# jyakaranda/A-LeGO-LOAM

Measured on AMD Instinct MI355X. Metric: scans/sec (16x1800 LiDAR) full IP->LO->LM loop, higher is better.
Workload: dtype f32/f64

## Files before the change

### a-lego-loam_amd/binding.py

```python
import ctypes as C
import os

import numpy as np

from .params import AlegoParams, AlegoPoint

_HERE = os.path.dirname(os.path.abspath(__file__))
_lib = None
_DT = {0: np.float32, 1: np.float64, 2: np.int32, 3: np.uint8}

EXPORTS = [
    "alego_create", "alego_destroy", "alego_last_error", "alego_device_count", "alego_params_sizeof",
    "alego_ip_process", "alego_lo_process", "alego_lm_process", "alego_scan_process",
    "alego_batch_load", "alego_batch_run", "alego_synchronize", "alego_batch_get_pose", "alego_batch_get_counts",
    "alego_stream", "alego_stream_groups", "alego_profile_enable", "alego_profile_report", "alego_set_lo_params", "alego_set_lm_params", "alego_debug_get", "alego_debug_voxel", "alego_debug_atan2f",
    "alego_lo_push_imu", "alego_lo_get_undistorted", "alego_pose_o2b", "alego_trajectory_enable", "alego_trajectory_get", "alego_debug_check_guards", "alego_debug_math", "alego_debug_std_sort", "alego_debug_eval_blocks", "alego_debug_transform_to_start", "alego_debug_set_option",
    "alego_lm_keyframe_count", "alego_lm_get_keyframe", "alego_lm_set_keypose", "alego_lm_reset_window", "alego_lm_apply_correction",
    "alego_lm_add_keyframe", "alego_pc2_to_points", "alego_replay_create", "alego_replay_load", "alego_replay_assign",
    "alego_dist_unique_id", "alego_dist_init", "alego_dist_shutdown", "alego_dist_allreduce_probe", "alego_stream_setup", "alego_stream_run",
    "alego_loop_detect", "alego_loop_closure_icp",
    "alego_bag_open", "alego_bag_close", "alego_bag_last_error", "alego_bag_topic_count", "alego_bag_topic_info", "alego_bag_message_count",
    "alego_bag_read_raw", "alego_bag_read_pc2", "alego_handle_lock", "alego_handle_unlock",
    "alego_map_enable", "alego_map_status", "alego_map_set_keyposes", "alego_map_get_keyframe", "alego_map_assemble", "alego_map_keyposes",
    "alego_lm_get_local_map", "alego_voxel_grid", "alego_write_pcd",
    "alego_map_get_stamps", "alego_map_set_stamps", "alego_loop_search", "alego_loop_constraint", "alego_debug_nn1",
    "alego_graph_enable", "alego_graph_status", "alego_graph_get_edges", "alego_graph_set_edges", "alego_graph_add_loops", "alego_graph_add_edge",
    "alego_graph_optimize", "alego_graph_get_estimate", "alego_graph_residuals",
    "alego_loc_select", "alego_loc_enable", "alego_loc_status",
    "alego_reloc_enable", "alego_loc_relocalize", "alego_reloc_descriptor", "alego_reloc_match", "alego_debug_reloc_search",
    "alego_loop_appearance_enable", "alego_loop_search_appearance", "alego_loop_appearance_candidates",
    "alego_map_align", "alego_map_align_queries", "alego_map_align_consensus", "alego_map_align_poses",
    "alego_map_move", "alego_map_merge", "alego_map_align_edge", "alego_map_merge_edges",
    "alego_map_thin", "alego_map_thin_select", "alego_map_thin_edges", "alego_debug_thin_select",
]

REPLAY_PINGPONG = 0x100
REPLAY_BAG = 0x200
MAP_SURF, MAP_CORNER, MAP_OUTLIER, MAP_FRAME_ID = 1, 2, 4, 8
ERR_CAPACITY, ERR_ARG = -3, -4
RELOC_MAX_CAND = 8
RELOC_SECTORS, RELOC_RINGS = 60, 20
ALIGN_MAX_QUERIES = 32
ALIGN_TOL_TRANS, ALIGN_TOL_ROT = 0.24, 0.0165
MERGE_COPY_ITEM = 1024
FLAG_LO_INIT, FLAG_FEW_SURF, FLAG_FEW_CORNER, FLAG_LM_SKIPPED, FLAG_LM_FEW_FEATURES, FLAG_LM_KEYFRAME = 1, 2, 4, 8, 16, 32


class ScanIn(C.Structure):
    _fields_ = [("pts", C.c_void_p), ("n", C.c_int32), ("stamp", C.c_double)]


class SegOut(C.Structure):
    _fields_ = [("seg", C.c_void_p), ("seg_cap", C.c_int32), ("m", C.c_int32),
                ("ground", C.c_void_p), ("col", C.c_void_p), ("range", C.c_void_p),
                ("ring_start", C.c_void_p), ("ring_end", C.c_void_p), ("orientation", C.c_float * 3),
                ("outlier", C.c_void_p), ("outlier_cap", C.c_int32), ("n_outlier", C.c_int32),
                ("label_image", C.c_void_p), ("stamp", C.c_double)]


class FeatOut(C.Structure):
    _fields_ = [("sharp", C.c_void_p), ("sharp_cap", C.c_int32), ("n_sharp", C.c_int32),
                ("less_sharp", C.c_void_p), ("less_sharp_cap", C.c_int32), ("n_less_sharp", C.c_int32),
                ("flat", C.c_void_p), ("flat_cap", C.c_int32), ("n_flat", C.c_int32),
                ("less_flat", C.c_void_p), ("less_flat_cap", C.c_int32), ("n_less_flat", C.c_int32),
                ("point_label", C.c_void_p)]


class Pose(C.Structure):
# ... 142 lines not shown


class Pc2Field(C.Structure):
    _fields_ = [("name", C.c_char_p), ("offset", C.c_uint32), ("datatype", C.c_uint8), ("count", C.c_uint32)]


def lib_path():
    return os.environ.get("ALEGO_LIB") or os.path.join(_HERE, "libalego_mi355x.so")


def lib():
    global _lib
    if _lib is None:
        path = lib_path()
        if not os.path.exists(path):
            raise RuntimeError(f"{path} missing: the HIP extension is not built (run __graft_entry__.build()); "
                               "there is no CPU fallback")
        L = C.CDLL(path)
        L.alego_create.restype = C.c_int
        L.alego_create.argtypes = [C.POINTER(AlegoParams), C.c_int, C.c_int, C.c_int, C.POINTER(C.c_void_p)]
        L.alego_destroy.argtypes = [C.c_void_p]
        L.alego_last_error.restype = C.c_char_p
        L.alego_last_error.argtypes = [C.c_void_p]
        L.alego_device_count.restype = C.c_int
        L.alego_params_sizeof.restype = C.c_int
        L.alego_ip_process.restype = C.c_int
        L.alego_ip_process.argtypes = [C.c_void_p, C.POINTER(ScanIn), C.POINTER(SegOut)]
        L.alego_lo_process.restype = C.c_int
        L.alego_lo_process.argtypes = [C.c_void_p, C.POINTER(SegOut), C.POINTER(FeatOut), C.POINTER(Pose)]
        L.alego_lm_process.restype = C.c_int
        L.alego_lm_process.argtypes = [C.c_void_p, C.c_void_p, C.c_int32, C.c_void_p, C.c_int32, C.c_void_p, C.c_int32,
                                       C.POINTER(Pose), C.POINTER(Pose)]
        L.alego_scan_process.restype = C.c_int
        L.alego_scan_process.argtypes = [C.c_void_p, C.c_int, C.POINTER(ScanIn), C.c_int, C.POINTER(SegOut),
                                         C.POINTER(FeatOut), C.POINTER(Pose), C.POINTER(Pose)]
        L.alego_batch_load.restype = C.c_int
        L.alego_batch_load.argtypes = [C.c_void_p, C.c_int, C.c_int, C.c_void_p, C.c_int32]
        L.alego_batch_run.restype = C.c_int
        L.alego_batch_run.argtypes = [C.c_void_p, C.c_int, C.c_int, C.c_int, C.c_int]
        L.alego_synchronize.restype = C.c_int
        L.alego_synchronize.argtypes = [C.c_void_p]
        L.alego_batch_get_pose.restype = C.c_int
        L.alego_batch_get_pose.argtypes = [C.c_void_p, C.c_int, C.POINTER(Pose), C.POINTER(Pose)]
        L.alego_batch_get_counts.restype = C.c_int
        L.alego_batch_get_counts.argtypes = [C.c_void_p, C.c_int, C.c_void_p, C.c_int]
        L.alego_profile_enable.restype = C.c_int
        L.alego_profile_enable.argtypes = [C.c_void_p, C.c_int]
        L.alego_profile_report.restype = C.c_int
        L.alego_profile_report.argtypes = [C.c_void_p, C.c_char_p, C.c_int, C.c_void_p, C.c_void_p, C.c_int]
        L.alego_stream.restype = C.c_void_p
        L.alego_stream.argtypes = [C.c_void_p]
        L.alego_stream_groups.restype = C.c_int
        L.alego_stream_groups.argtypes = [C.c_void_p, C.POINTER(C.c_int)]
        L.alego_set_lo_params.restype = C.c_int
        L.alego_set_lo_params.argtypes = [C.c_void_p, C.c_int, C.c_void_p]
        L.alego_set_lm_params.restype = C.c_int
        L.alego_set_lm_params.argtypes = [C.c_void_p, C.c_int, C.c_void_p]
        L.alego_debug_get.restype = C.c_int
        L.alego_debug_get.argtypes = [C.c_void_p, C.c_int, C.c_char_p, C.c_void_p, C.c_int, C.POINTER(C.c_int), C.POINTER(C.c_int)]
        L.alego_debug_voxel.restype = C.c_int
        L.alego_debug_voxel.argtypes = [C.c_void_p, C.c_void_p, C.c_int, C.c_float, C.c_void_p, C.c_int]
        L.alego_debug_atan2f.restype = C.c_int
        L.alego_debug_atan2f.argtypes = [C.c_void_p, C.c_void_p, C.c_void_p, C.c_void_p, C.c_int]
        L.alego_trajectory_enable.restype = C.c_int
        L.alego_trajectory_enable.argtypes = [C.c_void_p, C.c_int32]
        L.alego_trajectory_get.restype = C.c_int
        L.alego_trajectory_get.argtypes = [C.c_void_p, C.c_int, C.c_int32, C.c_int32, C.c_void_p]
        L.alego_lo_push_imu.restype = C.c_int
        L.alego_lo_push_imu.argtypes = [C.c_void_p, C.c_int, C.c_void_p, C.c_int32]
        L.alego_lo_get_undistorted.restype = C.c_int
        L.alego_lo_get_undistorted.argtypes = [C.c_void_p, C.c_int, C.c_void_p, C.c_int32]
        L.alego_pose_o2b.restype = C.c_int
        L.alego_pose_o2b.argtypes = [C.c_void_p, C.c_void_p, C.c_void_p]
        L.alego_debug_check_guards.restype = C.c_int
        L.alego_debug_check_guards.argtypes = [C.c_char_p, C.c_int]
        L.alego_debug_std_sort.restype = C.c_int
        L.alego_debug_std_sort.argtypes = [C.c_void_p, C.c_void_p, C.c_int, C.c_int, C.c_void_p]
        L.alego_debug_math.restype = C.c_int
        L.alego_debug_math.argtypes = [C.c_void_p, C.c_int, C.c_void_p, C.c_void_p, C.c_void_p, C.c_int]
        L.alego_debug_eval_blocks.restype = C.c_int
        L.alego_debug_eval_blocks.argtypes = [C.c_void_p, C.c_int, C.c_int, C.c_void_p, C.c_void_p, C.c_void_p, C.c_void_p]
        L.alego_debug_transform_to_start.restype = C.c_int
        L.alego_debug_transform_to_start.argtypes = [C.c_void_p, C.c_void_p, C.c_void_p, C.c_int, C.c_void_p]
        L.alego_debug_set_option.restype = C.c_int
        L.alego_debug_set_option.argtypes = [C.c_void_p, C.c_char_p, C.c_int]
        L.alego_lm_keyframe_count.restype = C.c_int
        L.alego_lm_keyframe_count.argtypes = [C.c_void_p, C.c_int]
        L.alego_lm_get_keyframe.restype = C.c_int
        L.alego_lm_get_keyframe.argtypes = [C.c_void_p, C.c_int, C.c_int, C.POINTER(KeyFrame)]
        L.alego_lm_set_keypose.restype = C.c_int
        L.alego_lm_set_keypose.argtypes = [C.c_void_p, C.c_int, C.c_int, C.c_void_p]
        L.alego_lm_reset_window.restype = C.c_int
        L.alego_lm_reset_window.argtypes = [C.c_void_p, C.c_int]
        L.alego_lm_apply_correction.restype = C.c_int
        L.alego_lm_apply_correction.argtypes = [C.c_void_p, C.c_int, C.c_void_p]
        L.alego_lm_add_keyframe.restype = C.c_int
        L.alego_lm_add_keyframe.argtypes = [C.c_void_p, C.c_int, C.c_void_p, C.c_void_p, C.c_int32, C.c_void_p, C.c_int32, C.c_void_p, C.c_int32]
        L.alego_pc2_to_points.restype = C.c_int
        L.alego_pc2_to_points.argtypes = [C.c_void_p, C.c_uint64, C.c_uint32, C.c_uint32, C.c_uint32, C.c_uint32, C.c_int,
                                          C.POINTER(Pc2Field), C.c_int, C.c_void_p, C.c_int32]
        L.alego_replay_create.restype = C.c_int
        L.alego_replay_create.argtypes = [C.c_void_p, C.c_int, C.c_int]
        L.alego_replay_load.restype = C.c_int
        L.alego_replay_load.argtypes = [C.c_void_p, C.c_int, C.c_int, C.c_void_p, C.c_int32]
        L.alego_replay_assign.restype = C.c_int
        L.alego_replay_assign.argtypes = [C.c_void_p, C.c_int, C.c_int, C.c_int]
# ... 479 lines not shown

    def replay_create(self, n_bags, bag_len):
        self._check(lib().alego_replay_create(self._h, n_bags, bag_len), "alego_replay_create")

    def replay_load(self, bag, scan, pts):
        a = np.ascontiguousarray(pts, dtype=np.float32)
        self._check(lib().alego_replay_load(self._h, bag, scan, a.ctypes.data, a.shape[0]), "alego_replay_load")

    def replay_assign(self, slot, bag, start_scan):
        self._check(lib().alego_replay_assign(self._h, slot, bag, start_scan), "alego_replay_assign")

    def stream_setup(self, bag, start_scan=0):
        self._check(lib().alego_stream_setup(self._h, bag, start_scan), "alego_stream_setup")

    def stream_run(self, first_step, n_scans, stages=7, sync=True):
        self._check(lib().alego_stream_run(self._h, first_step, n_scans, stages, 1 if sync else 0), "alego_stream_run")

    def batch_run(self, first_pos, n_scans, stages=7, sync=True):
        self._check(lib().alego_batch_run(self._h, first_pos, n_scans, stages, 1 if sync else 0), "alego_batch_run")

    def synchronize(self):
        self._check(lib().alego_synchronize(self._h), "alego_synchronize")

    def batch_get_pose(self, slot=0):
        odom, mp = Pose(), Pose()
        flags = self._check(lib().alego_batch_get_pose(self._h, slot, C.byref(odom), C.byref(mp)), "alego_batch_get_pose")
        return flags, odom.as_dict(), mp.as_dict()

    def batch_get_counts(self, slot=0):
        out = np.zeros(16, np.int32)
        self._check(lib().alego_batch_get_counts(self._h, slot, out.ctypes.data, 16), "alego_batch_get_counts")
        keys = ["P", "M", "O", "Qc", "Fc", "Qs", "Fs", "n_surf_corr", "n_corner_corr", "Kraw_c", "Kraw_s", "Kds_c", "Kds_s", "Lc", "Ls", "n_rebuild"]
        return dict(zip(keys, out.tolist()))

    def profile_enable(self, on=True):
        self._check(lib().alego_profile_enable(self._h, 1 if on else 0), "alego_profile_enable")

    def profile_report(self):
        names = C.create_string_buffer(8192)
        tot = np.zeros(256, np.float64)
        cnt = np.zeros(256, np.int32)
        n = self._check(lib().alego_profile_report(self._h, names, 8192, tot.ctypes.data, cnt.ctypes.data, 256), "alego_profile_report")
        ks = names.value.decode().split(";") if n else []
        return {k: (float(tot[i]), int(cnt[i])) for i, k in enumerate(ks)}

    def stream(self):
        return lib().alego_stream(self._h)

    def stream_groups(self):
        per = C.c_int(0)
        g = lib().alego_stream_groups(self._h, C.byref(per))
        return g, per.value

    def set_lo_params(self, p6, slot=0):
        a = np.ascontiguousarray(p6, np.float64)
        self._check(lib().alego_set_lo_params(self._h, slot, a.ctypes.data), "alego_set_lo_params")

    def set_lm_params(self, p6, slot=0):
        a = np.ascontiguousarray(p6, np.float64)
        self._check(lib().alego_set_lm_params(self._h, slot, a.ctypes.data), "alego_set_lm_params")

    def debug_get(self, name, slot=0, cap_bytes=None):
        cap = cap_bytes or max(self.N * 64 + 4096, 8 << 20)
        buf = np.empty(cap, np.uint8)
        cnt, dt = C.c_int(), C.c_int()
        self._check(lib().alego_debug_get(self._h, slot, name.encode(), buf.ctypes.data, cap, C.byref(cnt), C.byref(dt)),
                    f"alego_debug_get({name})")
        dtype = np.dtype(_DT[dt.value])
        out = np.frombuffer(buf.tobytes()[:cnt.value * dtype.itemsize], dtype=dtype).copy()
        return out.reshape(-1, 4) if (name in _CLOUDS or name.startswith("lm_") and name.endswith(("_ds", "_map"))) else out

    def voxel_grid(self, pts, leaf):
        a = np.ascontiguousarray(pts, np.float32)
        out = np.empty((max(a.shape[0], 1), 4), np.float32)
        n = self._check(lib().alego_debug_voxel(self._h, a.ctypes.data, a.shape[0], leaf, out.ctypes.data, out.shape[0]), "alego_debug_voxel")
        return out[:n].copy()

    def voxel_grid_large(self, pts, leaf):
        a = np.ascontiguousarray(pts, np.float32).reshape(-1, 4)
        n = self._check(lib().alego_voxel_grid(self._h, a.ctypes.data, a.shape[0], leaf, None, 0), "alego_voxel_grid")
        out = np.empty((max(n, 1), 4), np.float32)
        m = self._check(lib().alego_voxel_grid(self._h, a.ctypes.data, a.shape[0], leaf, out.ctypes.data, out.shape[0]), "alego_voxel_grid")
        return out[:m].copy()

    def map_enable(self, max_keyframes, max_points):
        self._check(lib().alego_map_enable(self._h, max_keyframes, max_points), "alego_map_enable")

    def map_status(self, slot=0):
        out = np.zeros(4, np.int32)
        self._check(lib().alego_map_status(self._h, slot, out.ctypes.data), "alego_map_status")
        return tuple(int(v) for v in out)

    def map_set_keyposes(self, first, poses6, slot=0):
        a = np.ascontiguousarray(poses6, np.float32).reshape(-1, 6)
        self._check(lib().alego_map_set_keyposes(self._h, slot, first, a.shape[0], a.ctypes.data), "alego_map_set_keyposes")

    def map_get_keyframe(self, kf_id, slot=0):
        k = KeyFrame()
        self._check(lib().alego_map_get_keyframe(self._h, slot, kf_id, C.byref(k)), "alego_map_get_keyframe")
        bufs = [np.empty((max(n, 1), 4), np.float32) for n in (k.n_corner, k.n_surf, k.n_outlier)]
        k.corner, k.corner_cap = bufs[0].ctypes.data, bufs[0].shape[0]
        k.surf, k.surf_cap = bufs[1].ctypes.data, bufs[1].shape[0]
        k.outlier, k.outlier_cap = bufs[2].ctypes.data, bufs[2].shape[0]
        self._check(lib().alego_map_get_keyframe(self._h, slot, kf_id, C.byref(k)), "alego_map_get_keyframe")
        return dict(id=int(k.id), pose=np.array(k.pose[:], np.float32), corner=bufs[0][:k.n_corner].copy(), surf=bufs[1][:k.n_surf].copy(),
                    outlier=bufs[2][:k.n_outlier].copy())
# ... 336 lines not shown
```

### a-lego-loam_amd/csrc/alego_api.hip

```cpp
#include <hip/hip_runtime.h>

#include <cmath>
#include <cstdio>
#include <cstdlib>
#include <algorithm>
#include <cstring>
#include <mutex>
#include <set>
#include <string>
#include <vector>

#include "../../include/alego_mi355x.h"
#include "dev_common.h"
#include "dev_mem.h"
#include "front_end.h"
#include "lm_ctx.h"
#include "lm_host.h"
#include "merge_math.h"
#include "thin_math.h"
#include "loop_ctx.h"
#include "pgraph.h"
#include "prof.h"
#include "reloc.h"
#include "voxel.h"

thread_local Profiler* g_prof = nullptr;


struct alego_handle {
  std::recursive_mutex host_lock;
  alego_params P;
  int device = 0;
  hipStream_t stream = nullptr;
  std::vector<hipStream_t> streams;
  int gsize = 1;
  bool lm_async = false;
  std::vector<hipStream_t> back;
  std::vector<hipEvent_t> ev_stage, ev_back;
  std::vector<long> grp_scans;
  DevCtx d;
  DevPool mem;
  std::string err;
  std::vector<long> lo_scans;
  LmHost* lm = nullptr;
  Profiler prof;
  int ip_fast_capable = 0;
  bool replay_assigned = false;
  bool stream_mode = false;
  int lanes = 0;
  int pose_slot = 0;
  int last_lane = -1;
  std::vector<double> imu_last_stamp;
  int next_set = 0;
  hipStream_t s_lo = nullptr, s_lm = nullptr;
  std::vector<hipEvent_t> ev_pool;
  size_t ev_next = 0;
  bool map_on = false;
  LcCtx* lc = nullptr;
  bool graph_on = false;
  PgCtx* pg = nullptr;
  RlCtx* rl = nullptr;
};

namespace {

#define HIP_TRY(h, call)                                                                       \
  do {                                                                                         \
    hipError_t e_ = (call);                                                                    \
    if (e_ != hipSuccess) {                                                                    \
      (h)->err = std::string(#call) + ": " + hipGetErrorString(e_);                            \
      return ALEGO_ERR_HIP;                                                                    \
    }                                                                                          \
  } while (0)

template <class T>
int dalloc(alego_handle* h, T** p, size_t count, bool zero = true) {
  const hipError_t e = h->mem.get(p, count, zero);
  if (e != hipSuccess) { h->err = std::string("device allocation: ") + hipGetErrorString(e); return ALEGO_ERR_HIP; }
  return 0;
}

DevCtx view(const alego_handle* h, int slot0, int n) {
  DevCtx d = h->d;
  d.slot0 = slot0;
  d.n_launch = n;
  return d;
}

hipStream_t stream_of(const alego_handle* h, int slot) { return h->streams[slot / h->gsize]; }
hipError_t sync_all(const alego_handle* h) {
  hipError_t r = hipSuccess;
  for (hipStream_t s : h->streams) { hipError_t e = hipStreamSynchronize(s); if (e != hipSuccess) r = e; }
  for (hipStream_t s : h->back) { hipError_t e = hipStreamSynchronize(s); if (e != hipSuccess) r = e; }
  for (hipStream_t s : {h->s_lo, h->s_lm}) if (s) { hipError_t e = hipStreamSynchronize(s); if (e != hipSuccess) r = e; }
  return r;
}

int env_int(const char* name, int dflt) { const char* e = getenv(name); return e ? atoi(e) : dflt; }

void drain_back(alego_handle* h, int slot = -1) {
  if (slot >= 0 && !h->back.empty()) { (void)hipStreamSynchronize(h->back[std::min<size_t>((size_t)(slot / h->gsize), h->back.size() - 1)]); return; }
  for (hipStream_t s : h->back) (void)hipStreamSynchronize(s);
}
int check_slot(alego_handle* h, int slot, bool drain = true) {
  if (!h) return ALEGO_ERR_ARG;
  if (slot < 0 || slot >= h->d.n_slots) { h->err = "slot out of range"; return ALEGO_ERR_ARG; }
  if (drain) drain_back(h, slot);
  return 0;
}

int not_localising(alego_handle* h, const char* what) {
  if (h->lm && lm_host_localising(h->lm)) { h->err = std::string(what) + ": not available on a localising handle (alego_loc_enable)"; return ALEGO_ERR_ARG; }
  return 0;
}

}

extern "C" {

int alego_device_count(void) {
  int n = 0;
  if (hipGetDeviceCount(&n) != hipSuccess) return 0;
  return n;
}
int alego_params_sizeof(void) { return (int)sizeof(alego_params); }
int alego_handle_lock(alego_handle* h) { if (!h) return ALEGO_ERR_ARG; h->host_lock.lock(); return 0; }
int alego_handle_unlock(alego_handle* h) { if (!h) return ALEGO_ERR_ARG; h->host_lock.unlock(); return 0; }
const char* alego_last_error(const alego_handle* h) { return h ? h->err.c_str() : "null handle"; }
void* alego_stream(alego_handle* h) { return h ? (void*)h->stream : nullptr; }
int alego_stream_groups(const alego_handle* h, int* slots_per_group) {
  if (!h) return ALEGO_ERR_ARG;
  if (slots_per_group) *slots_per_group = h->gsize;
  return (int)h->streams.size();
}

int alego_create(const alego_params* params, int device, int n_slots, int ring_len, alego_handle** out) {
  if (!params || !out) return ALEGO_ERR_ARG;
  *out = nullptr;
  int ndev = 0;
  if (hipGetDeviceCount(&ndev) != hipSuccess || ndev <= 0 || device < 0 || device >= ndev) return ALEGO_ERR_NO_DEVICE;
  hipDeviceProp_t prop;
  if (hipGetDeviceProperties(&prop, device) != hipSuccess) return ALEGO_ERR_NO_DEVICE;
  if (std::strncmp(prop.gcnArchName, "gfx950", 6) != 0) {
    std::fprintf(stderr, "alego_create: device %d is %s, this library is built for gfx950 only\n", device, prop.gcnArchName);
    return ALEGO_ERR_NO_DEVICE;
  }
  if (n_slots <= 0) n_slots = 1;
  if (ring_len <= 0) ring_len = 1;
  if (params->n_scan < 1 || params->n_scan > 64 || params->horizon_scan < 64 || params->horizon_scan > 4096) return ALEGO_ERR_ARG;
  if (params->sort_mode != 0 && params->sort_mode != 2) { std::fprintf(stderr, "alego_create: sort_mode %d is an oracle-only setting (0 = (curvature, index) order, 2 = libstdc++ std::sort tie order in the sector sort)\n", params->sort_mode); return ALEGO_ERR_ARG; }
  if (params->deskew_mode != 0 && params->deskew_mode != 1) { std::fprintf(stderr, "alego_create: deskew_mode must be 0 or 1\n"); return ALEGO_ERR_ARG; }
  if (params->deskew_mode && !(params->scan_period > 0)) { std::fprintf(stderr, "alego_create: scan_period must be positive\n"); return ALEGO_ERR_ARG; }
  if (params->kf_cap_surf < 0 || params->kf_cap_outlier < 0) { std::fprintf(stderr, "alego_create: negative key-frame capacity\n"); return ALEGO_ERR_ARG; }
  if (params->recent_keyframe_num > 512) { std::fprintf(stderr, "alego_create: recent_keyframe_num > 512 is not supported\n"); return ALEGO_ERR_ARG; }
  if (params->suppress_radius < 0 || params->suppress_radius > 5 || params->n_sectors < 1 || params->n_sharp < 0 ||
      params->n_less_sharp < params->n_sharp || params->n_flat < 1) {
    std::fprintf(stderr, "alego_create: feature-pick parameters out of range (0 <= suppress_radius <= 5, n_sectors >= 1, 0 <= n_sharp <= n_less_sharp, n_flat >= 1)\n");
    return ALEGO_ERR_ARG;
  }
  {
    const int sector_max = (params->horizon_scan + params->n_sectors - 1) / params->n_sectors + 2;
    if (sector_max > 64 * 12) {
      std::fprintf(stderr, "alego_create: ceil(horizon_scan / n_sectors) + 2 = %d exceeds the 768 sector elements the feature pick holds\n", sector_max);
      return ALEGO_ERR_ARG;
    }
  }
  alego_handle* h = new alego_handle();
  h->P = *params;
  h->device = device;
  h->lo_scans.assign(n_slots, 0);
  if (hipSetDevice(device) != hipSuccess) { delete h; return ALEGO_ERR_HIP; }
  {
    int G = n_slots / 64;
    if (const char* e = getenv("ALEGO_STREAM_GROUPS")) G = atoi(e);
    if (G > 8) G = 8;
    if (G > n_slots) G = n_slots;
    if (G < 1) G = 1;
    if (!getenv("ALEGO_STREAM_GROUPS") && G > 4) G = 4;
    h->gsize = (n_slots + G - 1) / G;
    G = (n_slots + h->gsize - 1) / h->gsize;
    for (int g = 0; g < G; ++g) {
      hipStream_t s = nullptr;
      if (hipStreamCreate(&s) != hipSuccess) { for (hipStream_t t : h->streams) hipStreamDestroy(t); delete h; return ALEGO_ERR_HIP; }
      h->streams.push_back(s);
    }
    h->stream = h->streams[0];
    h->lm_async = env_int("ALEGO_LM_ASYNC", 1) != 0;
    if (h->lm_async) {
      for (int g = 0; g < G; ++g) {
        hipStream_t s = nullptr;
        hipEvent_t e[4] = {nullptr, nullptr, nullptr, nullptr};
        bool ok = hipStreamCreate(&s) == hipSuccess;
        for (int k = 0; k < 4 && ok; ++k) ok = hipEventCreateWithFlags(&e[k], hipEventDisableTiming) == hipSuccess;
        if (!ok) { h->lm_async = false; break; }
        h->back.push_back(s);
        h->ev_stage.push_back(e[0]); h->ev_stage.push_back(e[1]); h->ev_back.push_back(e[2]); h->ev_back.push_back(e[3]);
      }
      h->grp_scans.assign(G, 0);
    }
  }
  DevCtx& d = h->d;
  std::memset(&d, 0, sizeof(d));
  d.P = *params;
  d.n_slots = n_slots; d.ring_len = ring_len; d.slot0 = 0; d.n_launch = n_slots;
  d.fs_cur = d.fs_last = -1;
  d.NS = params->n_scan; d.H = params->horizon_scan; d.N = d.NS * d.H; d.Pcap = d.N;
  d.cap_sharp = params->n_sharp * params->n_sectors;
  d.cap_lsharp = params->n_less_sharp * params->n_sectors;
  d.cap_flat = params->n_flat * params->n_sectors;
  d.st_stride = d.cap_sharp + d.cap_lsharp + d.cap_flat + d.H;
  d.sin_ax = std::sin(params->seg_alpha_x); d.cos_ax = std::cos(params->seg_alpha_x);
  d.sin_ay = std::sin(params->seg_alpha_y); d.cos_ay = std::cos(params->seg_alpha_y);
  {
    const double lo = params->sensor_mount_ang - params->ground_angle_thres, hi = params->sensor_mount_ang + params->ground_angle_thres;
    const bool ok = lo > -89.0 && hi < 89.0 && lo < hi;
    d.tan_g_lo = ok ? std::tan(lo * M_PI / 180.0) : std::nan("");
    d.tan_g_hi = ok ? std::tan(hi * M_PI / 180.0) : std::nan("");
  }
  d.h_magic = (unsigned)((1ull << 32) / (unsigned long long)d.H) + 1u;
  d.inv_res_x = 1.0 / params->ang_res_x; d.inv_res_y = 1.0 / params->ang_res_y;
  d.tan_theta = (params->seg_theta > 0.0 && params->seg_theta < 1.5) ? std::tan(params->seg_theta) : std::nan("");
  d.opt_ip_fused = env_int("ALEGO_IP_FUSED", 1) != 0;
  d.opt_ip_half = env_int("ALEGO_IP_HALF", 1) != 0;
  d.opt_cc_fused = env_int("ALEGO_CC_FUSED", 1) != 0;
  d.opt_cc_tile = env_int("ALEGO_CC_TILE", 1) != 0;
  d.opt_ip_band = env_int("ALEGO_IP_BAND", 1) != 0;
  d.opt_fe_pick1 = env_int("ALEGO_FE_PICK1", 0) != 0;
  d.opt_fe_fused = env_int("ALEGO_FE_FUSED", 1) != 0;
  d.opt_fe_cand = env_int("ALEGO_FE_CAND", 0);
  d.opt_lo_box_lds = env_int("ALEGO_LO_BOX_LDS", 1 << 20);
  d.opt_lo_grid = env_int("ALEGO_LO_GRID", 1) != 0;
  d.opt_fo_spin = env_int("ALEGO_FE_SPIN", 0);
  d.opt_fo_pad8 = env_int("ALEGO_FE_PAD8", 0) != 0;
  d.opt_map_merge = env_int("ALEGO_MAP_MERGE", 1) != 0;
  d.fcap[F_SHARP] = d.cap_sharp * d.NS; d.fcap[F_LSHARP] = d.cap_lsharp * d.NS; d.fcap[F_FLAT] = d.cap_flat * d.NS; d.fcap[F_LFLAT] = d.N;
  d.lo_qcap_surf = d.fcap[F_FLAT]; d.lo_qcap_corner = d.fcap[F_SHARP];
  d.lo_box_cap = (d.N + LO_CH - 1) / LO_CH + d.NS;
  const size_t B = n_slots, N = d.N, NS = d.NS;
  int rc = 0;
  rc |= dalloc(h, &d.in_pts, B * ring_len * d.Pcap, false);
// ... 104 lines not shown
  if (int r = check_slot(h, slot, false)) return r;
  if (ring_pos < 0 || ring_pos >= h->d.ring_len || n < 0 || (n > 0 && !pts)) { h->err = "ring_pos / n out of range or null points"; return ALEGO_ERR_ARG; }
  if (n > h->d.Pcap) { h->err = "scan larger than n_scan*horizon_scan"; return ALEGO_ERR_CAPACITY; }
  hipSetDevice(h->device);
  float4* dst = h->d.in_pts + ((size_t)slot * h->d.ring_len + ring_pos) * h->d.Pcap;
  if (n > 0) HIP_TRY(h, hipMemcpyAsync(dst, pts, (size_t)n * sizeof(alego_point), hipMemcpyHostToDevice, stream_of(h, slot)));
  HIP_TRY(h, hipMemcpyAsync(h->d.in_n + slot * h->d.ring_len + ring_pos, &n, sizeof(int), hipMemcpyHostToDevice, stream_of(h, slot)));
  HIP_TRY(h, hipStreamSynchronize(stream_of(h, slot)));
  return 0;
}

int alego_replay_create(alego_handle* h, int n_bags, int bag_len) {
  if (!h || n_bags < 1 || bag_len < 1) return ALEGO_ERR_ARG;
  if (h->d.bag_pts) { h->err = "alego_replay_create: the bag store exists already"; return ALEGO_ERR_ARG; }
  hipSetDevice(h->device);
  float4* pts = nullptr; int* cnt = nullptr; int2* src = nullptr;
  if (dalloc(h, &pts, (size_t)n_bags * bag_len * h->d.Pcap, false) || dalloc(h, &cnt, (size_t)n_bags * bag_len) || dalloc(h, &src, (size_t)h->d.n_slots)) return ALEGO_ERR_HIP;
  h->d.bag_pts = pts; h->d.bag_n = cnt; h->d.bag_src = src; h->d.n_bags = n_bags; h->d.bag_len = bag_len;
  return 0;
}
int alego_replay_load(alego_handle* h, int bag, int scan, const alego_point* pts, int32_t n) {
  if (!h || !h->d.bag_pts || bag < 0 || bag >= h->d.n_bags || scan < 0 || scan >= h->d.bag_len || n < 0 || (n > 0 && !pts)) return ALEGO_ERR_ARG;
  if (n > h->d.Pcap) { h->err = "scan larger than n_scan*horizon_scan"; return ALEGO_ERR_CAPACITY; }
  hipSetDevice(h->device);
  const size_t idx = (size_t)bag * h->d.bag_len + scan;
  HIP_TRY(h, hipMemcpy(const_cast<float4*>(h->d.bag_pts) + idx * h->d.Pcap, pts, (size_t)n * sizeof(alego_point), hipMemcpyHostToDevice));
  HIP_TRY(h, hipMemcpy(const_cast<int*>(h->d.bag_n) + idx, &n, sizeof(int), hipMemcpyHostToDevice));
  return 0;
}
int alego_replay_assign(alego_handle* h, int slot, int bag, int start_scan) {
  if (int r = check_slot(h, slot)) return r;
  if (!h->d.bag_pts || bag < 0 || bag >= h->d.n_bags || start_scan < 0) return ALEGO_ERR_ARG;
  hipSetDevice(h->device);
  const int2 v = make_int2(bag, start_scan % h->d.bag_len);
  HIP_TRY(h, hipMemcpy(const_cast<int2*>(h->d.bag_src) + slot, &v, sizeof(v), hipMemcpyHostToDevice));
  h->replay_assigned = true;
  return 0;
}

int alego_stream_setup(alego_handle* h, int bag, int start_scan) {
  if (!h) return ALEGO_ERR_ARG;
  if (int r = not_localising(h, "alego_stream_setup")) return r;
  if (!h->d.bag_pts || bag < 0 || bag >= h->d.n_bags || start_scan < 0) { h->err = "alego_stream_setup: needs alego_replay_create and a valid bag"; return ALEGO_ERR_ARG; }
  if (h->d.n_slots < 3 || h->streams.size() != 1) { h->err = "alego_stream_setup: the handle needs n_slots = 1 + 2 W >= 3 (one stream group)"; return ALEGO_ERR_ARG; }
  if (h->d.traj) { h->err = "alego_stream_setup: the per-scan pose log belongs to the batch path"; return ALEGO_ERR_ARG; }
  if (h->map_on) { h->err = "alego_stream_setup: the key-frame archive belongs to the batch / single-scan paths"; return ALEGO_ERR_ARG; }
  if (h->P.deskew_mode) { h->err = "alego_stream_setup: bags carry no stamps / IMU data; the motion de-skew runs through alego_scan_process / alego_lo_process"; return ALEGO_ERR_ARG; }
  hipSetDevice(h->device);
  const int W = (h->d.n_slots - 1) / 2;
  if (int r = alego_replay_assign(h, 0, bag, start_scan)) return r;
  for (int set = 0; set < 2; ++set)
    for (int j = 0; j < W; ++j)
      if (int r = alego_replay_assign(h, 1 + set * W + j, bag, start_scan + j)) return r;
  if (!h->s_lo && (hipStreamCreate(&h->s_lo) != hipSuccess || hipStreamCreate(&h->s_lm) != hipSuccess)) { h->err = "alego_stream_setup: hipStreamCreate failed"; return ALEGO_ERR_HIP; }
  h->stream_mode = true; h->lanes = W; h->pose_slot = 0; h->last_lane = -1; h->next_set = 0;
  return 0;
}

int alego_stream_run(alego_handle* h, int first_step, int n_scans, int stages, int sync) {
  if (!h) return ALEGO_ERR_ARG;
  if (!h->stream_mode) { h->err = "alego_stream_run: call alego_stream_setup first"; return ALEGO_ERR_ARG; }
  hipSetDevice(h->device);
  drain_back(h);
  g_prof = &h->prof;
  const int W = h->lanes;
  hipStream_t sA = h->streams[0], sB = h->s_lo, sC = h->s_lm;
  auto ev = [&]() -> hipEvent_t {
    if (h->ev_next == h->ev_pool.size()) { hipEvent_t e; (void)hipEventCreateWithFlags(&e, hipEventDisableTiming); h->ev_pool.push_back(e); }
    return h->ev_pool[h->ev_next++];
  };
  h->ev_next = 0;
  {
    hipEvent_t eb = ev(), ec = ev(), ea = ev();
    HIP_TRY(h, hipEventRecord(eb, sB)); HIP_TRY(h, hipEventRecord(ec, sC));
    HIP_TRY(h, hipStreamWaitEvent(sA, eb, 0)); HIP_TRY(h, hipStreamWaitEvent(sA, ec, 0));
    HIP_TRY(h, hipEventRecord(ea, sA)); HIP_TRY(h, hipStreamWaitEvent(sB, ea, 0)); HIP_TRY(h, hipStreamWaitEvent(sC, ea, 0));
  }
  hipEvent_t lm_done[2] = {nullptr, nullptr};
  hipEvent_t lo_first_done = nullptr;
  const bool do_lo = (stages & 2) != 0, do_lm = do_lo && (stages & 4);
  int g = 0;
  for (int base = 0; base < n_scans; base += W, ++g) {
    const int w = std::min(W, n_scans - base), set = h->next_set, lane0 = 1 + set * W;
    h->next_set ^= 1;
    if (lm_done[set]) HIP_TRY(h, hipStreamWaitEvent(sA, lm_done[set], 0));
    if (lo_first_done) HIP_TRY(h, hipStreamWaitEvent(sA, lo_first_done, 0));
    DevCtx dl = view(h, lane0, w);
    dl.replay_bag = 1;
    const int pos = (int)(((long long)first_step + base) % h->d.bag_len);
    if (stages & 1) launch_ip(dl, pos, false, sA);
    if (do_lo) launch_fe(dl, sA);
    hipEvent_t fe_done = ev();
    HIP_TRY(h, hipEventRecord(fe_done, sA));
    if (!do_lo) { h->pose_slot = lane0 + w - 1; continue; }
    HIP_TRY(h, hipStreamWaitEvent(sB, fe_done, 0));
    for (int j = 0; j < w; ++j) {
      DevCtx ds = view(h, 0, 1);
      ds.fs_cur = lane0 + j; ds.fs_last = h->last_lane >= 0 ? h->last_lane : lane0 + j;
      launch_lo(ds, sB);
      hipEvent_t lo_done = ev();
      HIP_TRY(h, hipEventRecord(lo_done, sB));
      if (j == 0) lo_first_done = lo_done;
      const bool odom_valid = h->lo_scans[0]++ > 0;
      if (do_lm) {
        HIP_TRY(h, hipStreamWaitEvent(sC, lo_done, 0));
        if (int r = lm_host_enqueue(h->lm, ds, std::vector<char>(1, odom_valid ? 1 : 0), &h->err, sC)) return r;
      }
      h->last_lane = lane0 + j;
      h->pose_slot = lane0 + j;
    }
    hipEvent_t done = ev();
    HIP_TRY(h, hipEventRecord(done, do_lm ? sC : sB));
    lm_done[set] = done;
  }
  HIP_TRY(h, hipGetLastError());
  if (sync) HIP_TRY(h, sync_all(h));
  return 0;
}

// ... 1131 lines not shown
```

### include/alego_mi355x.h

```cpp
#ifndef ALEGO_MI355X_H_
#define ALEGO_MI355X_H_

#include <stdint.h>

#include "alego_params.h"

#ifdef __cplusplus
extern "C" {
#endif

typedef struct alego_handle alego_handle;

enum {
  ALEGO_OK = 0,
  ALEGO_ERR_NO_DEVICE = -1,
  ALEGO_ERR_HIP = -2,
  ALEGO_ERR_CAPACITY = -3,
  ALEGO_ERR_ARG = -4
};
enum {
  ALEGO_FLAG_LO_INIT = 1,
  ALEGO_FLAG_FEW_SURF = 2,
  ALEGO_FLAG_FEW_CORNER = 4,
  ALEGO_FLAG_LM_SKIPPED = 8,
// ... 17 lines not shown
  float orientation[3];
  alego_point* outlier;  int32_t outlier_cap;  int32_t n_outlier;
  int32_t* label_image;
  double stamp;
} alego_seg_out;

typedef struct alego_feat_out {
  alego_point* sharp;       int32_t sharp_cap;       int32_t n_sharp;
  alego_point* less_sharp;  int32_t less_sharp_cap;  int32_t n_less_sharp;
  alego_point* flat;        int32_t flat_cap;        int32_t n_flat;
  alego_point* less_flat;   int32_t less_flat_cap;   int32_t n_less_flat;
  int32_t* point_label;
} alego_feat_out;

typedef struct alego_pose {
  double t[3];
  double q[4];
  double params[6];
  int32_t valid;
} alego_pose;

int alego_create(const alego_params* params, int device, int n_slots, int ring_len, alego_handle** out);
void alego_destroy(alego_handle* h);
const char* alego_last_error(const alego_handle* h);
int alego_device_count(void);
int alego_params_sizeof(void);
int alego_handle_lock(alego_handle* h);
int alego_handle_unlock(alego_handle* h);

int alego_ip_process(alego_handle* h, const alego_scan_in* in, alego_seg_out* out);
int alego_lo_process(alego_handle* h, const alego_seg_out* in, alego_feat_out* feat, alego_pose* odom);
int alego_lm_process(alego_handle* h, const alego_point* corner_last, int32_t n_corner,
                     const alego_point* surf_last, int32_t n_surf, const alego_point* outlier,
                     int32_t n_outlier, const alego_pose* odom, alego_pose* map_pose);
int alego_scan_process(alego_handle* h, int slot, const alego_scan_in* in, int stages,
                       alego_seg_out* seg, alego_feat_out* feat, alego_pose* odom, alego_pose* map_pose);

int alego_batch_load(alego_handle* h, int slot, int ring_pos, const alego_point* pts, int32_t n);
int alego_batch_run(alego_handle* h, int first_pos, int n_scans, int stages, int sync);
int alego_synchronize(alego_handle* h);
#define ALEGO_REPLAY_PINGPONG 0x100
#define ALEGO_REPLAY_BAG 0x200
int alego_replay_create(alego_handle* h, int n_bags, int bag_len);
int alego_replay_load(alego_handle* h, int bag, int scan, const alego_point* pts, int32_t n);
int alego_replay_assign(alego_handle* h, int slot, int bag, int start_scan);
int alego_stream_setup(alego_handle* h, int bag, int start_scan);
int alego_stream_run(alego_handle* h, int first_step, int n_scans, int stages, int sync);
int alego_batch_get_pose(alego_handle* h, int slot, alego_pose* odom, alego_pose* map_pose);
int alego_trajectory_enable(alego_handle* h, int32_t capacity_scans);
int alego_trajectory_get(alego_handle* h, int slot, int32_t first, int32_t n, double* out14);
int alego_batch_get_counts(alego_handle* h, int slot, int32_t* out, int cap);
void* alego_stream(alego_handle* h);
int alego_stream_groups(const alego_handle* h, int* slots_per_group);

int alego_profile_enable(alego_handle* h, int on);
int alego_profile_report(alego_handle* h, char* names, int names_cap, double* total_ms, int* launches, int cap);

typedef struct alego_imu {
  double stamp;
  double orientation[4];
  double linear_acceleration[3];
  double angular_velocity[3];
} alego_imu;
int alego_lo_push_imu(alego_handle* h, int slot, const alego_imu* samples, int32_t n);
int alego_lo_get_undistorted(alego_handle* h, int slot, alego_point* out, int32_t cap);
int alego_pose_o2b(const alego_pose* o2l, const double* tf_b2l, alego_pose* o2b);

int alego_set_lo_params(alego_handle* h, int slot, const double* p6);
int alego_set_lm_params(alego_handle* h, int slot, const double* p6);
int alego_debug_get(alego_handle* h, int slot, const char* name, void* out, int cap_bytes,
                    int* count, int* dtype);
int alego_debug_voxel(alego_handle* h, const alego_point* pts, int n, float leaf, alego_point* out, int cap);
int alego_debug_atan2f(alego_handle* h, const float* y, const float* x, float* out, int n);
int alego_debug_std_sort(alego_handle* h, const uint32_t* keys, int n, int depth_limit, int32_t* order);
int alego_debug_math(alego_handle* h, int mode, const float* a, const float* b, float* out, int n);
int alego_debug_eval_blocks(alego_handle* h, int type, int n, const double* geom13, const double* params6, double* res, double* jac6);
int alego_debug_transform_to_start(alego_handle* h, const double* params6, const alego_point* pts, int n, alego_point* out);
int alego_debug_check_guards(char* report, int cap);
int alego_debug_set_option(alego_handle* h, const char* name, int value);

typedef struct alego_keyframe {
  int32_t id;
  float pose[6];
  alego_point* corner;   int32_t corner_cap;   int32_t n_corner;
  alego_point* surf;     int32_t surf_cap;     int32_t n_surf;
  alego_point* outlier;  int32_t outlier_cap;  int32_t n_outlier;
} alego_keyframe;
int alego_lm_keyframe_count(alego_handle* h, int slot);
int alego_lm_get_keyframe(alego_handle* h, int slot, int kf_id, alego_keyframe* out);
int alego_lm_set_keypose(alego_handle* h, int slot, int kf_id, const float pose6[6]);
int alego_lm_reset_window(alego_handle* h, int slot);
int alego_lm_apply_correction(alego_handle* h, int slot, const double rc[12]);
int alego_lm_add_keyframe(alego_handle* h, int slot, const float pose6[6], const alego_point* corner, int32_t n_corner,
                          const alego_point* surf, int32_t n_surf, const alego_point* outlier, int32_t n_outlier);

int alego_map_enable(alego_handle* h, int32_t max_keyframes, int32_t max_points);
int alego_map_get_stamps(alego_handle* h, int slot, int32_t first, int32_t n, double* out);
int alego_map_set_stamps(alego_handle* h, int slot, int32_t first, int32_t n, const double* stamps);
int alego_map_status(alego_handle* h, int slot, int32_t out[4]);
int alego_map_set_keyposes(alego_handle* h, int slot, int32_t first, int32_t n, const float* poses6);
int alego_map_get_keyframe(alego_handle* h, int slot, int32_t id, alego_keyframe* out);
enum {
  ALEGO_MAP_SURF = 1,
  ALEGO_MAP_CORNER = 2,
  ALEGO_MAP_OUTLIER = 4,
  ALEGO_MAP_FRAME_ID = 8
// ... 204 lines not shown
```

Baseline: 445,400.

## Plan stream groups and lookahead streams around available hardware queues

Adds a stream planner that sizes the number of stream groups and decides whether LM runs asynchronously, based on the hardware queue count (default 4, or from env). In streaming mode it reuses existing streams (the main stream and the first back stream) for the LO/LM lookahead stages instead of always creating two extra streams. It also drops the drain_back call at the start of each stream run. The intent is to avoid oversubscribing hardware queues, where streams sharing a queue would serialize or add switching cost, and to remove a per-run drain. In exchange, sharing streams may reduce stage overlap, and dropping the drain could change ordering with pending back-stream work.

```diff
diff --git a/a-lego-loam_amd/binding.py b/a-lego-loam_amd/binding.py
--- a/a-lego-loam_amd/binding.py
+++ b/a-lego-loam_amd/binding.py
@@ -13,7 +13,7 @@
     "alego_create", "alego_destroy", "alego_last_error", "alego_device_count", "alego_params_sizeof",
     "alego_ip_process", "alego_lo_process", "alego_lm_process", "alego_scan_process",
     "alego_batch_load", "alego_batch_run", "alego_synchronize", "alego_batch_get_pose", "alego_batch_get_counts",
-    "alego_stream", "alego_stream_groups", "alego_profile_enable", "alego_profile_report", "alego_set_lo_params", "alego_set_lm_params", "alego_debug_get", "alego_debug_voxel", "alego_debug_atan2f",
+    "alego_stream", "alego_stream_groups", "alego_stream_plan", "alego_profile_enable", "alego_profile_report", "alego_set_lo_params", "alego_set_lm_params", "alego_debug_get", "alego_debug_voxel", "alego_debug_atan2f",
     "alego_lo_push_imu", "alego_lo_get_undistorted", "alego_pose_o2b", "alego_trajectory_enable", "alego_trajectory_get", "alego_debug_check_guards", "alego_debug_math", "alego_debug_std_sort", "alego_debug_eval_blocks", "alego_debug_transform_to_start", "alego_debug_set_option",
     "alego_lm_keyframe_count", "alego_lm_get_keyframe", "alego_lm_set_keypose", "alego_lm_reset_window", "alego_lm_apply_correction",
     "alego_lm_add_keyframe", "alego_pc2_to_points", "alego_replay_create", "alego_replay_load", "alego_replay_assign",
@@ -262,6 +262,8 @@
         L.alego_stream.argtypes = [C.c_void_p]
         L.alego_stream_groups.restype = C.c_int
         L.alego_stream_groups.argtypes = [C.c_void_p, C.POINTER(C.c_int)]
+        L.alego_stream_plan.restype = C.c_int
+        L.alego_stream_plan.argtypes = [C.c_void_p, C.POINTER(C.c_int)]
         L.alego_set_lo_params.restype = C.c_int
         L.alego_set_lo_params.argtypes = [C.c_void_p, C.c_int, C.c_void_p]
         L.alego_set_lm_params.restype = C.c_int
@@ -847,6 +849,11 @@
         g = lib().alego_stream_groups(self._h, C.byref(per))
         return g, per.value
 
+    def stream_plan(self):
+        out = (C.c_int * 4)()
+        self._check(lib().alego_stream_plan(self._h, out), "alego_stream_plan")
+        return dict(groups=out[0], slots_per_group=out[1], lm_async=bool(out[2]), hw_queues=out[3])
+
     def set_lo_params(self, p6, slot=0):
         a = np.ascontiguousarray(p6, np.float64)
         self._check(lib().alego_set_lo_params(self._h, slot, a.ctypes.data), "alego_set_lo_params")
diff --git a/a-lego-loam_amd/csrc/alego_api.hip b/a-lego-loam_amd/csrc/alego_api.hip
--- a/a-lego-loam_amd/csrc/alego_api.hip
+++ b/a-lego-loam_amd/csrc/alego_api.hip
@@ -22,6 +22,7 @@
 #include "pgraph.h"
 #include "prof.h"
 #include "reloc.h"
+#include "stream_plan.h"
 #include "voxel.h"
 
 thread_local Profiler* g_prof = nullptr;
@@ -53,6 +54,8 @@
   std::vector<double> imu_last_stamp;
   int next_set = 0;
   hipStream_t s_lo = nullptr, s_lm = nullptr;
+  hipStream_t sB = nullptr, sC = nullptr;
+  StreamPlan plan = {1, 1, 0, STREAM_PLAN_DEFAULT_QUEUES};
   std::vector<hipEvent_t> ev_pool;
   size_t ev_next = 0;
   bool map_on = false;
@@ -132,6 +135,12 @@
   if (!h) return ALEGO_ERR_ARG;
   if (slots_per_group) *slots_per_group = h->gsize;
   return (int)h->streams.size();
+}
+
+int alego_stream_plan(const alego_handle* h, int out[4]) {
+  if (!h || !out) return ALEGO_ERR_ARG;
+  out[0] = (int)h->streams.size(); out[1] = h->gsize; out[2] = h->lm_async ? 1 : 0; out[3] = h->plan.queues;
+  return 0;
 }
 
 int alego_create(const alego_params* params, int device, int n_slots, int ring_len, alego_handle** out) {
@@ -171,21 +180,18 @@
   h->lo_scans.assign(n_slots, 0);
   if (hipSetDevice(device) != hipSuccess) { delete h; return ALEGO_ERR_HIP; }
   {
-    int G = n_slots / 64;
-    if (const char* e = getenv("ALEGO_STREAM_GROUPS")) G = atoi(e);
-    if (G > 8) G = 8;
-    if (G > n_slots) G = n_slots;
-    if (G < 1) G = 1;
-    if (!getenv("ALEGO_STREAM_GROUPS") && G > 4) G = 4;
-    h->gsize = (n_slots + G - 1) / G;
-    G = (n_slots + h->gsize - 1) / h->gsize;
+    const char *eg = getenv("ALEGO_STREAM_GROUPS"), *ea = getenv("ALEGO_LM_ASYNC");
+    h->plan = stream_plan(n_slots, stream_plan_queues(getenv("ALEGO_HW_QUEUES"), getenv("GPU_MAX_HW_QUEUES")),
+                          eg ? std::max(atoi(eg), 0) : -1, ea ? (atoi(ea) != 0 ? 1 : 0) : -1);
+    h->gsize = h->plan.gsize;
+    const int G = h->plan.groups;
     for (int g = 0; g < G; ++g) {
       hipStream_t s = nullptr;
       if (hipStreamCreate(&s) != hipSuccess) { for (hipStream_t t : h->streams) hipStreamDestroy(t); delete h; return ALEGO_ERR_HIP; }
       h->streams.push_back(s);
     }
     h->stream = h->streams[0];
-    h->lm_async = env_int("ALEGO_LM_ASYNC", 1) != 0;
+    h->lm_async = h->plan.async != 0;
     if (h->lm_async) {
       for (int g = 0; g < G; ++g) {
         hipStream_t s = nullptr;
@@ -396,7 +402,18 @@
   for (int set = 0; set < 2; ++set)
     for (int j = 0; j < W; ++j)
       if (int r = alego_replay_assign(h, 1 + set * W + j, bag, start_scan + j)) return r;
-  if (!h->s_lo && (hipStreamCreate(&h->s_lo) != hipSuccess || hipStreamCreate(&h->s_lm) != hipSuccess)) { h->err = "alego_stream_setup: hipStreamCreate failed"; return ALEGO_ERR_HIP; }
+  {
+    std::vector<hipStream_t> pool(1, h->streams[0]);
+    if (!h->back.empty()) pool.push_back(h->back[0]);
+    const size_t want = (size_t)stream_plan_lookahead_streams(h->plan.queues, (int)pool.size());
+    for (hipStream_t* own : {&h->s_lo, &h->s_lm}) {
+      if (pool.size() >= want) break;
+      if (!*own && hipStreamCreate(own) != hipSuccess) { h->err = "alego_stream_setup: hipStreamCreate failed"; return ALEGO_ERR_HIP; }
+      pool.push_back(*own);
+    }
+    if (pool.size() >= 3) { h->sC = h->back.empty() ? pool[2] : pool[1]; h->sB = h->back.empty() ? pool[1] : pool[2]; }
+    else h->sB = h->sC = pool.back();
+  }
   h->stream_mode = true; h->lanes = W; h->pose_slot = 0; h->last_lane = -1; h->next_set = 0;
   return 0;
 }
@@ -405,10 +422,9 @@
   if (!h) return ALEGO_ERR_ARG;
   if (!h->stream_mode) { h->err = "alego_stream_run: call alego_stream_setup first"; return ALEGO_ERR_ARG; }
   hipSetDevice(h->device);
-  drain_back(h);
   g_prof = &h->prof;
   const int W = h->lanes;
-  hipStream_t sA = h->streams[0], sB = h->s_lo, sC = h->s_lm;
+  hipStream_t sA = h->streams[0], sB = h->sB, sC = h->sC;
   auto ev = [&]() -> hipEvent_t {
     if (h->ev_next == h->ev_pool.size()) { hipEvent_t e; (void)hipEventCreateWithFlags(&e, hipEventDisableTiming); h->ev_pool.push_back(e); }
     return h->ev_pool[h->ev_next++];
diff --git a/a-lego-loam_amd/csrc/stream_plan.h b/a-lego-loam_amd/csrc/stream_plan.h
--- /dev/null
+++ b/a-lego-loam_amd/csrc/stream_plan.h
@@ -0,0 +1,60 @@
+#pragma once
+
+#include <cstdlib>
+
+struct StreamPlan {
+  int groups;
+  int gsize;
+  int async;
+  int queues;
+};
+
+constexpr int STREAM_PLAN_MAX_GROUPS = 8;
+constexpr int STREAM_PLAN_DEFAULT_GROUPS = 4;
+constexpr int STREAM_PLAN_FULL_QUEUES = 8;
+constexpr int STREAM_PLAN_DEFAULT_QUEUES = 4;
+
+constexpr int kGroupCap[STREAM_PLAN_FULL_QUEUES] = {1, 1, 2, 3, 4, 4, 4, 4};
+
+inline int stream_plan_queues(const char* alego_hw_queues, const char* gpu_max_hw_queues) {
+  const char* const src[2] = {alego_hw_queues, gpu_max_hw_queues};
+  for (const char* e : src) {
+    if (!e) continue;
+    const int q = std::atoi(e);
+    if (q >= 1) return q;
+  }
+  return STREAM_PLAN_DEFAULT_QUEUES;
+}
+
+inline void stream_plan_cover(int n_slots, int G, StreamPlan* p) {
+  if (G > n_slots) G = n_slots;
+  if (G < 1) G = 1;
+  p->gsize = (n_slots + G - 1) / G;
+  p->groups = (n_slots + p->gsize - 1) / p->gsize;
+}
+
+inline StreamPlan stream_plan(int n_slots, int Q, int req_groups, int req_async) {
+  StreamPlan p;
+  if (n_slots < 1) n_slots = 1;
+  if (Q < 1) Q = 1;
+  p.queues = Q;
+  int G;
+  if (req_groups >= 0) {
+    G = req_groups > STREAM_PLAN_MAX_GROUPS ? STREAM_PLAN_MAX_GROUPS : req_groups;
+  } else {
+    G = n_slots / 64;
+    if (G > STREAM_PLAN_DEFAULT_GROUPS) G = STREAM_PLAN_DEFAULT_GROUPS;
+    if (G < 1) G = 1;
+    int cap = Q < STREAM_PLAN_FULL_QUEUES ? kGroupCap[Q] : STREAM_PLAN_DEFAULT_GROUPS;
+    if (req_async > 0 && cap > Q / 2) cap = Q / 2 > 1 ? Q / 2 : 1;
+    if (G > cap) G = cap;
+  }
+  stream_plan_cover(n_slots, G, &p);
+  p.async = req_async >= 0 ? (req_async != 0) : (2 * p.groups <= Q);
+  return p;
+}
+
+inline int stream_plan_lookahead_streams(int Q, int have) {
+  int want = Q < 3 ? (Q < 1 ? 1 : Q) : 3;
+  return want > have ? want : have;
+}
diff --git a/include/alego_mi355x.h b/include/alego_mi355x.h
--- a/include/alego_mi355x.h
+++ b/include/alego_mi355x.h
@@ -93,6 +93,7 @@
 int alego_batch_get_counts(alego_handle* h, int slot, int32_t* out, int cap);
 void* alego_stream(alego_handle* h);
 int alego_stream_groups(const alego_handle* h, int* slots_per_group);
+int alego_stream_plan(const alego_handle* h, int out[4]);
 
 int alego_profile_enable(alego_handle* h, int on);
 int alego_profile_report(alego_handle* h, char* names, int names_cap, double* total_ms, int* launches, int cap);
```

Result: faster. 473,600, median of 6 (+6.3%).
